# acg-team/ProGraphMSA

Hardware: AMD Instinct MI355X
Metric: DP cell-updates/sec (GCUPS) + wall-clock on 256 seqs × 1000 aa, WAG (higher is better)
Workload: dtype f32

## Files before the change

prographmsa_amd/csrc/pgm_align_kernels.h:

```cpp
#ifndef PGM_ALIGN_KERNELS_H_
#define PGM_ALIGN_KERNELS_H_

#include <hip/hip_runtime.h>
#include <math.h>
#include <type_traits>
#include "pgm_device.h"

#define PGM_NEG_INF (-INFINITY)

__device__ __forceinline__ float pgm_ls_log_add(float x, float add) {
    const float a = 2.44247459618085927548717403238913328776812604856113966238617812902399112761292613763080658235564f;
    const float b = -4.2040783745848554315883301529007786406310628696382695994938550046831869207082846248658671f;
    const float c = -0.72123729809042963774358701619456664388406302428056983119308906451199556380646306f;
    const uint32_t bits = __float_as_uint(x);
    const float e = (float)((int32_t)(bits >> 23) - 126);
    const float d = __uint_as_float(((bits << 9) >> 9) ^ 0x3f000000u);
    float t = __fdiv_rn(b, __fsub_rn(d, c));
    const float u = __fadd_rn(e, a);
    t = __fadd_rn(t, add);
    t = __fadd_rn(t, u);
    return t;
}

__device__ __forceinline__ float pgm_emission_finish(float num, float ay, float bx, float match_init) {
    float q = __fdiv_rn(num, __fmul_rn(ay, bx));
    if (q != q) q = __uint_as_float(0xFFC00000u);
    return pgm_ls_log_add(q, match_init);
}

template <int DMAX, int NODES>
__global__ void __launch_bounds__(NODES) pgm_prep_kernel(const PgmJob *__restrict__ jobs, int *__restrict__ sync, uint32_t sync_ints) {
    extern __shared__ float prep_lds[];
    {
        const uint32_t nthreads = gridDim.x * gridDim.y * gridDim.z * NODES;
        const uint32_t gid = ((blockIdx.z * gridDim.y + blockIdx.y) * gridDim.x + blockIdx.x) * NODES + threadIdx.x;
        for (uint32_t i = gid; i < sync_ints; i += nthreads) sync[i] = 0;
    }
    const PgmJob &J = jobs[blockIdx.x];
    const bool first = blockIdx.y == 0;
    const uint32_t n = first ? J.n1 : J.n2;
    const uint32_t v0 = blockIdx.z * NODES;
    if (v0 >= n) return;
    if (J.tabhdr && J.tabhdr[0] == 0) {
        const uint32_t nc = J.dim + 2u;
        bool any = n - 1u >= v0 && n - 1u < v0 + (uint32_t)NODES;
        for (uint32_t c = 0; c < nc; ++c) {
            const uint32_t r = (uint32_t)J.tabhdr[1u + (first ? 0u : nc) + c];
            any = any || (r != 0u && r - 1u >= v0 && r - 1u < v0 + (uint32_t)NODES);
        }
        if (!any) return;
    }
    const uint32_t D = J.dim, DP = J.dp, ST = D + 1;
    float *Mf = prep_lds;
    float *pif = prep_lds + D * D;
    float *nl = pif + D;
    const uint32_t nn = min((uint32_t)NODES, n - v0);
    {
        const int32_t *pp = first ? J.pp1 : J.pp2;
        const uint32_t *pc = first ? J.pc1 : J.pc2, *pu = first ? J.pu1 : J.pu2;
        const float *pv = first ? J.pv1 : J.pv2;
        PgmTbNode *rec = (first ? J.tb1 : J.tb2) + v0;
        for (uint32_t i = threadIdx.x; i < nn * PGM_TB_PK; i += NODES) {
            const uint32_t node = i / PGM_TB_PK, k = i % PGM_TB_PK;
            const int32_t eb = pp[v0 + node];
            const uint32_t cnt = (uint32_t)(pp[v0 + node + 1] - eb);
            const int32_t e = cnt == 0u ? 0 : eb + (int32_t)min(k, cnt - 1u);
            if (k == 0) rec[node].cnt = cnt;
            rec[node].c[k] = pc[e]; rec[node].v[k] = pv[e]; rec[node].u[k] = pu[e];
        }
    }
    if (!first) for (uint32_t i = threadIdx.x; i < D * D; i += NODES) Mf[i] = (float)J.M[i];
    for (uint32_t i = threadIdx.x; i < D; i += NODES) pif[i] = (float)J.pi[i];
    const double *sites = first ? J.sites1 : J.sites2;
    const uint32_t *smap = first ? J.smap1 : J.smap2;
// ... 68 lines not shown
        bool same = true;
        float vs = 0.f;
        const float g0 = (float)col[0];
        for (uint32_t k = 0; k < D; ++k) {
            const float g = (float)col[k];
            if (g != 0.0f) { ++nz; sym = k; vs = g; }
            same = same && g == g0;
        }
        uint32_t c = 255u;
        if (nz == 0u) c = D + 1u;
        else if (nz == 1u && vs == 1.0f) c = sym;
        else if (same && g0 == uni) c = D;
        cls[v] = (uint8_t)c;
        if (c == 255u) atomicOr(J.tabhdr, 1);
        else atomicCAS(J.tabhdr + 1 + (first ? 0u : D + 2u) + c, 0, (int)v + 1);
    }
}

__device__ __forceinline__ size_t pgm_cell_index(const PgmJob &J, uint32_t y, uint32_t x) {
    const uint32_t b = y / PGM_ROWS, l = PGM_HALO + (y - b * PGM_ROWS);
    return ((size_t)b * J.tsteps + (x + l)) * 64u + l;
}
__device__ __forceinline__ float4 pgm_load_cell(const PgmJob &J, uint32_t y, uint32_t x) {
    return J.cells[pgm_cell_index(J, y, x)];
}

__device__ __forceinline__ float pgm_dpp_wave_shr1(float src, float lane0_value) {
    return __int_as_float(__builtin_amdgcn_update_dpp(__float_as_int(lane0_value), __float_as_int(src), 0x138, 0xf, 0xf, false));
}

#define PGM_GLOBAL __attribute__((address_space(1)))
typedef float pgm_v4f __attribute__((ext_vector_type(4)));
template <class T> __device__ __forceinline__ T pgm_gld(const T *p) { return *(const PGM_GLOBAL T *)(uintptr_t)p; }
#define PGM_EM_TB 4
template <int DP, int RB>
__global__ void __launch_bounds__(4 * PGM_ROWS) pgm_emission_skew_kernel(const PgmJob *__restrict__ jobs) {
    typedef float pgm_v2f __attribute__((ext_vector_type(2)));
    constexpr int NT = DP / 4;
    constexpr int COLS = 64 + PGM_EM_TB * PGM_BLOCK - PGM_HALO - 1;
    constexpr int STR = DP + 1;
    __shared__ pgm_v2f tp[(COLS + 1) * STR];
    __shared__ float bq[COLS];
    const PgmJob &J = jobs[blockIdx.z];
    const uint32_t tb0 = blockIdx.x * PGM_EM_TB;
    const uint32_t rsh = J.rshift, nvb = J.nb << rsh;
    if (tb0 >= J.nblk || 4u * RB * blockIdx.y >= nvb) return;
    if (J.tabhdr && pgm_gld(J.tabhdr) == 0) return;
    auto row_of = [&](uint32_t v, uint32_t lane_) { return ((((v >> rsh) << 6) + lane_) << rsh) | (v & ((1u << rsh) - 1u)); };
    auto sblock_of = [&](uint32_t v, uint32_t tb_) { return ((((size_t)(v >> rsh) * J.nblk + tb_) << rsh) | (v & ((1u << rsh) - 1u))); };
    const uint32_t t0 = tb0 * PGM_BLOCK;
    const int cbase = (int)t0 - 63;
    if (DP == 20 && RB == 1) {
        float *const tab = (float *)tp;
        static_assert(COLS * 21 <= (COLS + 1) * STR * 2, "score table must fit the column staging area");
        __shared__ float As[32];
        const uint32_t fb0 = 4u * blockIdx.y + threadIdx.x / PGM_ROWS;
        const uint32_t fl = threadIdx.x % PGM_ROWS;
        const bool active = fb0 < nvb;
        int sym = 20;
        bool plain = true;
        float a_row = 0.f;
        if (active) {
            const uint32_t y = row_of(fb0, fl);
            const uint32_t yc = (y + 1 < J.n1) ? y : 0u;
            const float4 *src = (const float4 *)(J.g1f + (size_t)DP * yc);
            int nz = 0;
#pragma unroll
            for (int q = 0; q < NT; ++q) {
                const float4 v = src[q];
                const float vv[4] = {v.x, v.y, v.z, v.w};
#pragma unroll
                for (int u = 0; u < 4; ++u)
                    if (vv[u] != 0.0f) { ++nz; sym = 4 * q + u; plain = plain && vv[u] == 1.0f; }
            }
            plain = plain && nz <= 1;
            a_row = J.a1[yc];
        }
        if (threadIdx.x < 32) As[threadIdx.x] = 0.f;
        if (__syncthreads_and(plain ? 1 : 0)) {
            if (active) As[sym] = a_row;
            __syncthreads();
            const float mi = J.sc.match_init;
            constexpr int NE = (COLS * 21 + 4 * PGM_ROWS - 1) / (4 * PGM_ROWS);
            float tt[NE], tb2[NE];
#pragma unroll
            for (int e = 0; e < NE; ++e) {
                const int i = (int)threadIdx.x + e * 4 * PGM_ROWS;
                const int ci = i / 21, k = i % 21, c = cbase + ci;
                const bool in = i < COLS * 21 && c >= 0 && c <= (int)J.ncol;
                tb2[e] = in ? J.b2[c] : 0.f;
                tt[e] = (in && k < 20) ? J.t2[(size_t)DP * c + k] : 0.f;
            }
#pragma unroll
            for (int e = 0; e < NE; ++e) {
                const int i = (int)threadIdx.x + e * 4 * PGM_ROWS;
                if (i < COLS * 21) tab[i] = pgm_emission_finish(0.0f + tt[e], As[i % 21], tb2[e], mi);
            }
            __syncthreads();
            if (!active) return;
            PGM_GLOBAL pgm_v4f *const Sq = (PGM_GLOBAL pgm_v4f *)(uintptr_t)J.S;
            const int l = PGM_HALO + (int)fl;
#pragma unroll 1
            for (int w = 0; w < PGM_EM_TB; ++w) {
                const uint32_t tb = tb0 + w;
                if (tb >= J.nblk) break;
                float out[PGM_BLOCK];
#pragma unroll
                for (int i = 0; i < PGM_BLOCK; ++i) out[i] = tab[((int)(tb * PGM_BLOCK) + i - l - cbase) * 21 + sym];
                PGM_GLOBAL pgm_v4f *dst = Sq + (sblock_of(fb0, tb) * 64u + (uint32_t)l) * (PGM_BLOCK / 4);
#pragma unroll
                for (int q = 0; q < PGM_BLOCK / 4; ++q) dst[q] = pgm_v4f{out[4 * q], out[4 * q + 1], out[4 * q + 2], out[4 * q + 3]};
            }
            return;
        }
    }
    const float4 *t2q = (const float4 *)J.t2;
    float *tpf = (float *)tp;
    for (int i = threadIdx.x; i < (COLS + 1) * NT; i += 4 * PGM_ROWS) {
        const int ci = i / NT, q = i % NT, c = cbase + ci;
        float4 v = make_float4(0.f, 0.f, 0.f, 0.f);
        if (c >= 0 && c <= (int)J.ncol) v = t2q[(size_t)NT * c + q];
        const float vv[4] = {v.x, v.y, v.z, v.w};
#pragma unroll
        for (int u = 0; u < 4; ++u) {
            const int k = 4 * q + u;
            if (ci < COLS) tpf[2 * (ci * STR + k)] = vv[u];
            if (ci > 0) tpf[2 * ((ci - 1) * STR + k) + 1] = vv[u];
        }
    }
    for (int i = threadIdx.x; i < COLS; i += 4 * PGM_ROWS) {
        const int col = cbase + i;
        bq[i] = (col >= 0 && col <= (int)J.ncol) ? J.b2[col] : 0.f;
    }
    __syncthreads();
    const uint32_t b0 = (4u * blockIdx.y + threadIdx.x / PGM_ROWS) * RB;
    const int l = PGM_HALO + (int)(threadIdx.x % PGM_ROWS);
    if (b0 >= nvb) return;
    float gy[RB][DP], ay[RB];
#pragma unroll
    for (int r = 0; r < RB; ++r) {
        const uint32_t y = row_of(b0 + (uint32_t)r, (uint32_t)(l - PGM_HALO));
        const uint32_t yc = (y + 1 < J.n1) ? y : 0u;
        const float4 *src = (const float4 *)(J.g1f + (size_t)DP * yc);
#pragma unroll
        for (int q = 0; q < NT; ++q) {
            const float4 v = src[q];
            gy[r][4 * q] = v.x; gy[r][4 * q + 1] = v.y; gy[r][4 * q + 2] = v.z; gy[r][4 * q + 3] = v.w;
        }
        ay[r] = J.a1[yc];
    }
    const float mi = J.sc.match_init;
    const uint32_t nblk = J.nblk;
    PGM_GLOBAL pgm_v4f *const Sq = (PGM_GLOBAL pgm_v4f *)(uintptr_t)J.S;
#pragma unroll 1
    for (int w = 0; w < PGM_EM_TB; ++w) {
        const uint32_t tb = tb0 + w;
        if (tb >= nblk) break;
        float out[RB][PGM_BLOCK];
#pragma unroll
        for (int i = 0; i < PGM_BLOCK; i += 2) {
            const int ci = (int)(tb * PGM_BLOCK) + i - l - cbase;
            const pgm_v2f *tc = tp + ci * STR;
            pgm_v2f acc[RB];
#pragma unroll
            for (int r = 0; r < RB; ++r) acc[r] = pgm_v2f{0.0f, 0.0f};
#pragma unroll
            for (int k = 0; k < DP; ++k) {
                const pgm_v2f tk = tc[k];
#pragma unroll
                for (int r = 0; r < RB; ++r) {
                    const pgm_v2f g = {gy[r][k], gy[r][k]};
                    acc[r] = acc[r] + g * tk;
                }
            }
#pragma unroll
            for (int r = 0; r < RB; ++r) {
                out[r][i] = pgm_emission_finish(acc[r].x, ay[r], bq[ci], mi);
                out[r][i + 1] = pgm_emission_finish(acc[r].y, ay[r], bq[ci + 1], mi);
            }
        }
#pragma unroll
        for (int r = 0; r < RB; ++r) {
            if (b0 + (uint32_t)r < nvb) {
                PGM_GLOBAL pgm_v4f *dst = Sq + (sblock_of(b0 + (uint32_t)r, tb) * 64u + (uint32_t)l) * (PGM_BLOCK / 4);
#pragma unroll
                for (int q = 0; q < PGM_BLOCK / 4; ++q) dst[q] = pgm_v4f{out[r][4 * q], out[r][4 * q + 1], out[r][4 * q + 2], out[r][4 * q + 3]};
            }
        }
// ... 2263 lines not shown
```

prographmsa_amd/csrc/pgm_capi.hip:

```cpp
#include <hip/hip_runtime.h>

#include <algorithm>
#include <cmath>
#include <cstdio>
#include <thread>
#include <atomic>
#include <chrono>
#include <queue>
#include <cstdlib>
#include <cstring>
#include <numeric>
#include <mutex>
#include <string>
#include <unordered_set>
#include <vector>
#include <sys/mman.h>

#include "pgm_align_kernels.h"
#include "pgm_crit_kernels.h"
#include "pgm_nw_kernels.h"
#include "pgm_csprofile_kernels.h"
#include "pgm_dist_kernels.h"
#include "pgm_merge_kernels.h"
#include "pgm_pool.h"
// ... 65 lines not shown
    if (reg) { (void)hipHostUnregister(p); free(p); }
    else (void)hipHostFree(p);
}
static void slot_free(int slot, void *p) {
    if (slot == pgm_ctx::C_HIN) pinned_free(p);
    else if (slot == pgm_ctx::C_HOST) (void)hipHostFree(p);
    else (void)hipFree(p);
}

struct Arena {
    uint8_t *base = nullptr;
    size_t off = 0, end = 0;
    bool overflow = false;
    size_t put(const void *src, size_t bytes, size_t align = 16) {
        const size_t o = (off + align - 1) / align * align;
        if (o + bytes > end) { overflow = true; return 0; }
        off = o + bytes;
        if (src && bytes) memcpy(base + o, src, bytes);
        return o;
    }
};
struct DevLayout {
    size_t bytes = 0;
    size_t take(size_t b, size_t align = 256) {
        size_t off = (bytes + align - 1) / align * align;
        bytes = off + b;
        return off;
    }
};

struct pgm_align_batch {
    uint32_t njobs = 0;
    uint64_t cells = 0;
    uint32_t maxdim = 0, maxnb = 0, maxn = 0;
    std::vector<PgmJob> jobs;
    std::vector<uint32_t> order;
    uint8_t *d_in = nullptr;
    uint8_t *d_work = nullptr;
    uint8_t *d_cells = nullptr;
    uint8_t *d_out = nullptr;
    size_t cap[8] = {0, 0, 0, 0, 0, 0, 0, 0};
    uint8_t *h_out = nullptr;
    uint8_t *h_in = nullptr;
    int *h_flag = nullptr;
    uint8_t *d_small = nullptr;
    uint8_t *d_S = nullptr;
    int *d_sync = nullptr;
    size_t sync_ints = 0, s_bytes = 0;
    PgmItem *d_items = nullptr;
    uint32_t *d_lean = nullptr;
    uint32_t nlean = 0, nlean_workers = 0;
    uint32_t nbands = 0, nband_workers = 0;
    uint32_t nbands_narrow = 0, nwide_workers = 0;
    PgmItem *d_bands = nullptr;
    unsigned long long *d_times = nullptr;
    hipEvent_t ev_join_b = nullptr;
    bool crit_c3 = false, rest_c3 = false;
    uint32_t ncrit = 0, ncrit_workers = 0, ntb_c = 0;
    hipEvent_t ev_join_c = nullptr;
    uint32_t ntb_b = 0, ntb_b_workers = 0;
    uint32_t lq_off = 0, ntb = 0, ntb_workers = 0;
    int2 *d_tblist = nullptr;
    hipEvent_t ev_fork = nullptr, ev_join = nullptr;
    uint32_t test_spin_limit = 0, test_stall_job = 0xFFFFFFFFu, test_stall_band = 0;
    double acc_ms[3] = {0, 0, 0};
    uint32_t acc_n = 0;
    bool ev_pending = false;
    uint32_t nitems = 0;
    uint32_t nworkers = 0, maxnblk = 0;
    PgmJob *d_jobs = nullptr;
    uint32_t *d_order = nullptr;
    int *d_tabhdr = nullptr;
    size_t in_bytes = 0, work_bytes = 0, cell_bytes = 0, out_bytes = 0;
    std::vector<size_t> res_off, map1_off, map2_off;
    hipEvent_t ev[5] = {nullptr, nullptr, nullptr, nullptr, nullptr};
};

extern "C" {

const char *pgm_last_error(void) { return g_err.c_str(); }

int pgm_device_count(void) {
    int n = 0;
    if (hipGetDeviceCount(&n) != hipSuccess) return 0;
    return n;
}

__global__ void pgm_warm_kernel() {}

int pgm_ctx_create(int device, pgm_ctx **out) {
    if (!out) return fail(PGM_ERR_INVALID, "null out");
    *out = nullptr;
    int n = 0;
    HIPCHK(hipGetDeviceCount(&n));
    if (device < 0 || device >= n) return fail(PGM_ERR_DEVICE, "no such HIP device");
    HIPCHK(hipSetDevice(device));
    pgm_ctx *c = new pgm_ctx;
    c->device = device;
    HIPCHK(hipGetDeviceProperties(&c->prop, device));
    HIPCHK(hipStreamCreateWithFlags(&c->stream, hipStreamNonBlocking));
    HIPCHK(hipStreamCreateWithFlags(&c->stream2, hipStreamNonBlocking));
    HIPCHK(hipStreamCreateWithFlags(&c->stream3, hipStreamNonBlocking));
    {
        int lo = 0, hi = 0;
// ... 361 lines not shown
    const double w = std::min(1.0, std::max(0.0, (rsweep / t_par - 1.0) / 0.5));
    r.fl = 1.0 - 0.4 * w; r.fb = 1.0 - 0.25 * w;
    auto need = [](double cost, double t, uint32_t most) { return (uint32_t)std::min<double>(most, std::max(1.0, std::ceil(cost / t))); };
    const uint32_t band_most = (nbands + PGM_WAVES - 1) / PGM_WAVES;
    uint32_t lean = nlean ? need(lean_cost, r.fl * r.t_goal, nlean) : 0u, band = nbands ? need(band_cost, r.fb * r.t_goal, band_most) : 0u;
    uint32_t rest = nrest ? need(rest_cost, r.t_goal, nrest) : 0u;
    if (lean + band + rest > cap) {
        const double scale = (double)cap / (double)(lean + band + rest);
        auto cut = [&](uint32_t v) { return v ? std::max(1u, (uint32_t)std::floor(v * scale)) : 0u; };
        lean = cut(lean); band = cut(band); rest = cut(rest);
        while (lean + band + rest > cap) {
            uint32_t *big = &rest; if (band > *big) big = &band; if (lean > *big) big = &lean;
            if (*big <= 1u) break;
            --*big;
        }
    }
    r.rest_need = rest;
    const uint32_t left = cap > lean + band + rest ? cap - lean - band - rest : 0u;
    if (nrest) rest = std::min(nrest, rest + left);
    else if (nbands) band = std::min(band_most, band + left);
    else if (nlean) lean = std::min(nlean, lean + left);
    r.lean = lean; r.band = band; r.rest = rest;
    return r;
}

static hipError_t classify_lean_jobs(pgm_ctx *ctx, pgm_align_batch *b) {
    if (!b->d_tabhdr || b->njobs == 0) return hipSuccess;
    hipError_t e = hipMemsetAsync(b->d_tabhdr, 0, 4 * (size_t)PGM_TAB_HDR * b->njobs, ctx->stream);
    if (e != hipSuccess) return e;
    hipLaunchKernelGGL(pgm_classify_kernel, dim3(b->njobs, 2, (b->maxn + 1023) / 1024), dim3(256), 0, ctx->stream, b->d_jobs);
    return hipGetLastError();
}

#define PGM_STATUS_PENDING 0x7ffffff0
static hipError_t launch_all(pgm_ctx *ctx, pgm_align_batch *b, bool timed) {
    hipStream_t s = ctx->stream;
    hipError_t e;
    for (uint32_t i = 0; i < b->njobs; ++i) ((PgmJob::Result *)(b->h_out + b->res_off[i]))->status = PGM_STATUS_PENDING;
    if (timed && (e = hipEventRecord(b->ev[0], s)) != hipSuccess) return e;
    if (b->maxdim <= 20) {
        const size_t prep_lds = ((size_t)b->maxdim * b->maxdim + b->maxdim + 256 * ((size_t)b->maxdim + 1)) * sizeof(float);
        hipLaunchKernelGGL((pgm_prep_kernel<20, 256>), dim3(b->njobs, 2, (b->maxn + 255) / 256), dim3(256), prep_lds, s, b->d_jobs, b->d_sync, (uint32_t)b->sync_ints);
    } else {
        const size_t prep_lds = ((size_t)b->maxdim * b->maxdim + b->maxdim + 64 * ((size_t)b->maxdim + 1)) * sizeof(float);
        hipLaunchKernelGGL((pgm_prep_kernel<64, 64>), dim3(b->njobs, 2, (b->maxn + 63) / 64), dim3(64), prep_lds, s, b->d_jobs, b->d_sync, (uint32_t)b->sync_ints);
    }
    if ((e = hipGetLastError()) != hipSuccess) return e;
    if (timed && (e = hipEventRecord(b->ev[1], s)) != hipSuccess) return e;
    const dim3 eg((b->maxnblk + PGM_EM_TB - 1) / PGM_EM_TB, (b->maxnb + 3) / 4, b->njobs);
    if (b->maxdim <= 20) hipLaunchKernelGGL((pgm_emission_skew_kernel<20, 1>), eg, dim3(4 * PGM_ROWS), 0, s, b->d_jobs);
    else hipLaunchKernelGGL((pgm_emission_skew_kernel<64, 1>), eg, dim3(4 * PGM_ROWS), 0, s, b->d_jobs);
    if ((e = hipGetLastError()) != hipSuccess) return e;
    if (timed && (e = hipEventRecord(b->ev[2], s)) != hipSuccess) return e;
    const uint32_t spin_limit = b->test_spin_limit ? b->test_spin_limit : PGM_SPIN_LIMIT, stall_job = b->test_stall_job, stall_band = b->test_stall_band;
    const bool fork = b->nlean != 0;
    const bool bandk = b->nbands != 0;
    const bool tbk = (b->nitems != 0 || bandk) && (b->ntb + b->ntb_c + b->ntb_b) != 0;
    const bool critk = b->ncrit != 0;
    if ((fork || bandk || critk) && (e = hipEventRecord(b->ev_fork, s)) != hipSuccess) return e;
    if (critk && (e = hipStreamWaitEvent(ctx->stream4, b->ev_fork, 0)) != hipSuccess) return e;
    if (fork && (e = hipStreamWaitEvent(ctx->stream2, b->ev_fork, 0)) != hipSuccess) return e;
    if (bandk && (e = hipStreamWaitEvent(ctx->stream3, b->ev_fork, 0)) != hipSuccess) return e;
    const uint32_t nrest = b->nitems - b->ncrit;
    hipStream_t sc = critk ? s : ctx->stream4, sr = critk ? ctx->stream4 : s;
    auto sweep = [&](hipStream_t st, uint32_t workers, const PgmItem *list, uint32_t n, bool c3, uint32_t ticket_off) {
        if (c3) hipLaunchKernelGGL(pgm_crit_kernel, dim3(workers), dim3(64 * PGM_C3_WAVES), 0, st, b->d_jobs, list, n, b->d_sync, spin_limit, stall_job, stall_band, ticket_off);
        else hipLaunchKernelGGL(pgm_fill_kernel, dim3(workers), dim3(64 * PGM_WAVES), 0, st, b->d_jobs, list, n, b->d_sync, spin_limit, stall_job, stall_band, ticket_off);
    };
    auto tracebacks = [&](hipStream_t st, uint32_t workers, uint32_t first, uint32_t n, uint32_t lq_off, uint32_t sybase) {
        hipLaunchKernelGGL(pgm_tb_kernel, dim3(workers), dim3(64 * PGM_WAVES), 0, st, b->d_jobs, b->d_tblist + first, n, b->d_sync, b->test_spin_limit, lq_off, sybase, 1u);
    };
    if (critk) sweep(sc, b->ncrit_workers, b->d_items, b->ncrit, b->crit_c3, (uint32_t)PGM_SY_CRIT_TICKET);
    if (nrest != 0) sweep(sr, b->nworkers, b->d_items + b->ncrit, nrest, b->rest_c3, 1u);
    if ((e = hipGetLastError()) != hipSuccess) return e;
    if (fork) {
        hipLaunchKernelGGL((pgm_lean_kernel<2>), dim3(b->nlean_workers), dim3(64 * PGM_WAVES), 0, ctx->stream2, b->d_jobs, b->d_lean, b->nlean, b->d_sync, spin_limit);
        if ((e = hipGetLastError()) != hipSuccess) return e;
    }
    const uint32_t njp = (b->njobs + 3u) / 4u * 4u;
    if (bandk) {
        hipLaunchKernelGGL(pgm_band_kernel, dim3(b->nband_workers), dim3(64 * PGM_WAVES), 0, ctx->stream3, b->d_jobs, b->d_bands, b->nbands_narrow, b->nbands, b->nband_workers - b->nwide_workers, b->d_sync, spin_limit, stall_job, stall_band);
        if ((e = hipGetLastError()) != hipSuccess) return e;
        if (tbk && b->ntb_b) tracebacks(ctx->stream3, b->ntb_b_workers, b->ntb + b->ntb_c, b->ntb_b, b->lq_off + njp, 8u);
        if ((e = hipGetLastError()) != hipSuccess) return e;
// ... 56 lines not shown
        size_t E = (size_t)std::max(0, g->e_rowptr ? g->e_rowptr[n] : 0);
        if (g->r_rowptr) E += (size_t)std::max(0, g->r_rowptr[n]);
        const size_t full = side_bound_bytes(n, g->dim, E);
        return (res && res->dev_sites) ? full - n * g->dim * 8 + n * 4 + 16 : full;
    };
    auto ref_of = [&](const pgm_site_ref *r, uint32_t i) -> const pgm_site_ref * { return (r && r[i].dev_sites) ? &r[i] : nullptr; };
    std::vector<size_t> in_base(njobs + 1, 0);
    std::vector<char> two_chains(njobs, 0);
    (void)lib_pool().run(njobs, njobs >= 16 ? 16u : 1u, [&](size_t i) {
        const pgm_graph *a = g1[i], *c = g2[i];
        two_chains[i] = (a && c && a->n >= 2 && c->n >= 2 && a->e_rowptr && c->e_rowptr && a->e_col && c->e_col && a->e_val && c->e_val && graph_is_chain(a) && graph_is_chain(c)) ? 1 : 0;
    });
    uint32_t batch_dim = 0;
    for (uint32_t i = 0; i < njobs; ++i) if (g1[i]) batch_dim = std::max(batch_dim, g1[i]->dim);
    const uint32_t batch_dp = batch_dim <= 20 ? 20u : 64u;
    for (uint32_t i = 0; i < njobs; ++i) {
        const pgm_graph *a = g1[i], *c = g2[i];
        if (!a || !c || !model[i] || a->dim != c->dim || a->dim == 0 || a->dim > PGM_MAX_DIM || a->n < 2 || c->n < 2 || !model[i]->M || !model[i]->pi ||
            (!a->sites && !ref_of(res1, i)) || !a->e_rowptr || (!c->sites && !ref_of(res2, i)) || !c->e_rowptr) {
            delete b;
            return fail(PGM_ERR_INVALID, "invalid job " + std::to_string(i));
        }
        PgmJob &J = b->jobs[i];
        memset(&J, 0, sizeof J);
        J.n1 = a->n; J.n2 = c->n; J.dim = a->dim;
        J.dp = batch_dp;
        J.ncol = c->n - 1;
        J.tsteps = J.ncol + 63;
        constexpr uint32_t lean_rshift = 1u;
        J.lean = (two_chains[i] && ((uint64_t)J.tsteps * 1024u << lean_rshift) < (1ull << 30)) ? 1u : 0u;
        J.rshift = J.lean ? lean_rshift : 0u;
        J.nb = (a->n - 1 + (PGM_ROWS << J.rshift) - 1) / (PGM_ROWS << J.rshift);
        J.nblk = (J.tsteps + PGM_BLOCK - 1) / PGM_BLOCK;
        b->maxnblk = std::max(b->maxnblk, J.nblk);
        J.maxn = std::max(a->n, c->n);
        b->maxn = std::max(b->maxn, J.maxn);
        J.sc = scores[i];
        b->maxdim = std::max(b->maxdim, a->dim);
        b->maxnb = std::max(b->maxnb, J.nb << J.rshift);
        b->cells += (uint64_t)(a->n - 2) * (c->n - 2);
        Off &o = off[i];
        in_base[i + 1] = in_base[i] + side_bound(a, ref_of(res1, i)) + side_bound(c, ref_of(res2, i)) + model_bound_bytes(a->dim);
        J.keep_cells = (!J.lean || (flags & PGM_BATCH_KEEP_MATRICES)) ? 1u : 0u;
        layout_job(L, J.n1, J.n2, J.dp, J.rshift, J.lean != 0, J.keep_cells != 0, o);
        b->res_off[i] = o.res; b->map1_off[i] = o.map1; b->map2_off[i] = o.map2;
    }
    b->in_bytes = std::max<size_t>(in_base[njobs], 16);
    b->work_bytes = std::max<size_t>(L.W.bytes, 16);
    b->cell_bytes = std::max<size_t>(L.C.bytes, 16);
    b->out_bytes = std::max<size_t>(L.O.bytes, 16);
    b->s_bytes = std::max<size_t>(L.SL.bytes, 16);
    b->lq_off = (uint32_t)L.sync_ints;
    L.sync_ints += 3 * (((size_t)njobs + 3) / 4 * 4);
    const size_t sync_ints = L.sync_ints;
    b->sync_ints = sync_ints;
    hipError_t alloc_err = hipSuccess, alloc_host_err = hipSuccess;
    uint8_t *h_out_dev = nullptr;
    const bool cprof = getenv("PGM_HOST_PROFILE") != nullptr;
    auto now_ms = []() { return std::chrono::duration<double, std::milli>(std::chrono::steady_clock::now().time_since_epoch()).count(); };
    const double tc0 = now_ms();
    double tc_alloc = 0, tc_hostalloc = 0, tc_slot[6] = {0, 0, 0, 0, 0, 0};
    size_t total_bands = 0;
    for (uint32_t i = 0; i < njobs; ++i) total_bands += b->jobs[i].nb;
    DevLayout SM;
    const size_t small_sync = SM.take(sync_ints * sizeof(int)), small_jobs = SM.take(sizeof(PgmJob) * std::max(1u, njobs)),
                 small_order = SM.take(4 * (size_t)std::max(1u, njobs)), small_items = SM.take(sizeof(PgmItem) * std::max<size_t>(1, total_bands)),
                 small_lean = SM.take(4 * (size_t)std::max(1u, njobs)), small_tblist = SM.take(8 * (size_t)std::max(1u, njobs)),
                 small_bands = SM.take(sizeof(PgmItem) * std::max<size_t>(1, total_bands)), small_times = SM.take(16 * (size_t)std::max(1u, njobs) + 16);
    bool any_lean = false;
    for (uint32_t i = 0; i < njobs; ++i) any_lean = any_lean || (b->jobs[i].lean && !b->jobs[i].keep_cells);
    const size_t small_tabhdr = SM.take(any_lean ? 4 * (size_t)PGM_TAB_HDR * njobs : 16);
    const size_t small_bytes = SM.bytes;
    std::atomic<int> alloc_state(0);
    std::atomic<int> upload_err((int)hipSuccess);
    std::thread alloc_thread([&]() {
        const double ta0 = now_ms();
        hipError_t e2 = hipSetDevice(ctx->device);
        double tprev = ta0;
        auto lap = [&](int k) { const double t = now_ms(); tc_slot[k] = t - tprev; tprev = t; };
        if (e2 == hipSuccess) { e2 = cache_take(ctx, pgm_ctx::C_IN, b->in_bytes, (void **)&b->d_in, &b->cap[pgm_ctx::C_IN]); lap(0); }
        if (e2 == hipSuccess) { e2 = cache_take(ctx, pgm_ctx::C_WORK, b->work_bytes, (void **)&b->d_work, &b->cap[pgm_ctx::C_WORK]); lap(1); }
        if (e2 == hipSuccess) { e2 = cache_take(ctx, pgm_ctx::C_CELLS, b->cell_bytes, (void **)&b->d_cells, &b->cap[pgm_ctx::C_CELLS]); lap(2); }
        if (e2 == hipSuccess) { e2 = cache_take(ctx, pgm_ctx::C_OUT, b->out_bytes, (void **)&b->d_out, &b->cap[pgm_ctx::C_OUT]); lap(3); }
        if (e2 == hipSuccess) { e2 = cache_take(ctx, pgm_ctx::C_S, b->s_bytes, (void **)&b->d_S, &b->cap[pgm_ctx::C_S]); lap(4); }
        if (e2 == hipSuccess) { e2 = cache_take(ctx, pgm_ctx::C_SMALL, small_bytes, (void **)&b->d_small, &b->cap[pgm_ctx::C_SMALL]); lap(5); }
        if (e2 == hipSuccess) {
            b->d_sync = (int *)(b->d_small + small_sync);
            b->d_jobs = (PgmJob *)(b->d_small + small_jobs);
            b->d_order = (uint32_t *)(b->d_small + small_order);
            b->d_items = (PgmItem *)(b->d_small + small_items);
            b->d_lean = (uint32_t *)(b->d_small + small_lean);
            b->d_tblist = (int2 *)(b->d_small + small_tblist);
            b->d_bands = (PgmItem *)(b->d_small + small_bands);
            b->d_times = (unsigned long long *)(b->d_small + small_times);
            b->d_tabhdr = any_lean ? (int *)(b->d_small + small_tabhdr) : nullptr;
        }
        alloc_err = e2;
        alloc_state.store(e2 == hipSuccess ? 1 : -1, std::memory_order_release);
        tc_alloc = now_ms() - ta0;
        if (e2 == hipSuccess) {
            hipError_t e3 = cache_take(ctx, pgm_ctx::C_HOST, b->out_bytes + 64, (void **)&b->h_out, &b->cap[pgm_ctx::C_HOST]);
            if (e3 == hipSuccess) b->h_flag = (int *)(b->h_out + (b->out_bytes + 15) / 16 * 16);
            if (e3 == hipSuccess) e3 = hipHostGetDevicePointer((void **)&h_out_dev, b->h_out, 0);
            alloc_host_err = e3;
        }
        tc_hostalloc = now_ms() - ta0 - tc_alloc;
    });
    hipError_t e;
    if ((e = cache_take(ctx, pgm_ctx::C_HIN, b->in_bytes, (void **)&b->h_in, &b->cap[pgm_ctx::C_HIN])) != hipSuccess) {
        alloc_thread.join();
        pgm_align_batch_destroy(ctx, b);
        return fail(PGM_ERR_DEVICE, std::string("hipHostMalloc: ") + hipGetErrorString(e));
    }
    const double tc1 = now_ms();
    {
        std::atomic<int> bad(-1);
        constexpr uint32_t mode2_min_bands = 20u, mode2_min_hd = 32u;
        double longest_crit_chain = 0.0;
        for (uint32_t i = 0; i < njobs; ++i)
            longest_crit_chain = std::max(longest_crit_chain, ((double)((g1[i]->n - 1 + PGM_ROWS - 1) / PGM_ROWS - 1) * 80.0 + (double)(g2[i]->n - 1 + 63)) * 0.42);
        uint32_t promote_bands = 0xffffffffu;
        {
            double crit_load = 0.0;
            for (uint32_t i = 0; i < njobs; ++i)
                if (!b->jobs[i].lean) crit_load += (double)((g1[i]->n - 1 + PGM_ROWS - 1) / PGM_ROWS) * (double)(g2[i]->n - 1 + 63) * 0.42;
            if (crit_load <= 1.25 * (double)ctx->prop.multiProcessorCount * longest_crit_chain) promote_bands = 8u;
        }
        const uint32_t chunk_jobs = (uint32_t)std::max<size_t>(1, ((size_t)8 << 20) / std::max<size_t>(1, in_base[njobs] / std::max(1u, njobs)));
// ... 98 lines not shown
        J.ni1 = (const PgmNode2 *)(in + o.s1.ni); J.ni2 = (const PgmNode2 *)(in + o.s2.ni);
        J.xp1 = (const int32_t *)(in + o.s1.xp); J.xp2 = (const int32_t *)(in + o.s2.xp);
        J.xc1 = (const uint32_t *)(in + o.s1.xc); J.xc2 = (const uint32_t *)(in + o.s2.xc);
        J.xv1 = (const float *)(in + o.s1.xv); J.xv2 = (const float *)(in + o.s2.xv);
        J.fp1 = (const int32_t *)(in + o.s1.fp); J.fe1 = (const uint2 *)(in + o.s1.fe);
        J.ov2 = (const uint2 *)(in + o.s2.ov);
        J.pp1 = (const int32_t *)(in + o.s1.pp); J.pp2 = (const int32_t *)(in + o.s2.pp);
        J.pc1 = (const uint32_t *)(in + o.s1.pc); J.pc2 = (const uint32_t *)(in + o.s2.pc);
        J.pv1 = (const float *)(in + o.s1.pv); J.pv2 = (const float *)(in + o.s2.pv);
        J.pu1 = (const uint32_t *)(in + o.s1.pu); J.pu2 = (const uint32_t *)(in + o.s2.pu);
        J.g1f = (float *)(w + o.g1f); J.a1 = (float *)(w + o.a1);
        J.t2 = (float *)(w + o.t2); J.b2 = (float *)(w + o.aux2);
        J.map1 = (uint32_t *)(ob + o.map1); J.map2 = (uint32_t *)(ob + o.map2);
        J.mark_score = (float *)(w + o.ms); J.mark_prev = (uint32_t *)(w + o.mp);
        J.tb1 = (PgmTbNode *)(w + o.tb1); J.tb2 = (PgmTbNode *)(w + o.tb2);
        J.result = (PgmJob::Result *)(ob + o.res);
        J.hmap1 = (uint32_t *)(h_out_dev + o.map1); J.hmap2 = (uint32_t *)(h_out_dev + o.map2);
        J.hresult = (PgmJob::Result *)(h_out_dev + o.res);
        J.cells = (float4 *)(b->d_cells + o.cells);
        J.codes = (uint32_t *)(w + o.codes);
        J.endcell = (float4 *)(w + o.endcell);
        if (J.lean && !J.keep_cells && b->d_tabhdr) { J.cls1 = w + o.cls; J.cls2 = w + o.cls + J.n1; J.tabhdr = b->d_tabhdr + (size_t)PGM_TAB_HDR * i; }
        else { J.cls1 = nullptr; J.cls2 = nullptr; J.tabhdr = nullptr; }
        J.S = (float *)(b->d_S + o.S);
        J.prog = b->d_sync + o.prog;
        J.ltab = (uint16_t *)(w + o.ltab); J.lready = b->d_sync + o.lready; J.lrows = o.lrows; J.lcols = o.lcols;
        J.times = b->d_times + 2 * (size_t)i;
    }
    b->order.resize(njobs);
    std::iota(b->order.begin(), b->order.end(), 0u);
    std::stable_sort(b->order.begin(), b->order.end(), [&](uint32_t x, uint32_t y) {
        return (uint64_t)b->jobs[x].n1 * b->jobs[x].n2 > (uint64_t)b->jobs[y].n1 * b->jobs[y].n2;
    });
    std::vector<PgmItem> items;
    std::vector<uint32_t> lean_list;
    double lean_cost = 0.0, other_cost = 0.0;
    uint32_t capacity = (uint32_t)ctx->prop.multiProcessorCount;
    std::vector<PgmItem> bands;
    if (njobs) {
        struct Item { double rem, dur, gap; uint32_t job, band, count; };
        std::vector<std::vector<Item>> per_job(njobs), per_job_b(njobs), per_job_c(njobs), per_job_w(njobs);
        std::vector<double> chain_of(njobs, 0.0);
        const double lag = PGM_ROWS + 3.0 * PGM_BLOCK;
        constexpr double tau_x = 0.65, tau_c = 0.45, tau_2 = 0.6, eager = 0.7;
        constexpr double tau_3 = 0.42;
        constexpr double tau_l = 0.34;
        size_t total = 0, total_b = 0, total_w = 0;
        double rmax = 1.0, rsweep = 1.0;
        for (uint32_t q = 0; q < njobs; ++q) {
            const uint32_t i = b->order[q];
            const PgmJob &J = b->jobs[i];
            const double tau = J.crit3 ? tau_3 : (J.mode2 ? tau_2 : (J.has_extras ? tau_x : tau_c));
            const double tb = (J.has_extras ? 0.3 : 0.2) * (double)(J.n1 + J.n2);
            if (J.lean) {
                const double rounds = std::ceil((double)J.nb / PGM_WAVES), first = std::min<double>(J.nb, PGM_WAVES);
                lean_cost += tau_l * (rounds * J.tsteps + (first - 1.0) * 72.0) + 0.04 * (double)(J.n1 + J.n2);
                lean_list.push_back(i);
                continue;
            }
            const bool narrow = !J.mode2 && J.slot_bytes <= (uint32_t)(PGM_POOL / PGM_WAVES / 16 * 16);
            const bool wide = !J.mode2 && !narrow && J.slot_bytes <= (uint32_t)(PGM_POOL / PGM_WIDE_WAVES / 16 * 16);
            const bool per_band = narrow || wide;
            if (!per_band) chain_of[i] = tau * ((double)(J.nb - 1) * lag + J.tsteps);
            const uint32_t group = per_band ? 1u : J.nslots;
            for (uint32_t band = 0; band < J.nb; band += group) {
                const uint32_t cnt = std::min(group, J.nb - band);
// ... 141 lines not shown
    b->nworkers = std::max(1u, std::min(capacity, b->nitems - b->ncrit));
    b->crit_c3 = b->ncrit != 0; b->rest_c3 = b->nitems > b->ncrit;
    for (size_t k = 0; k < items.size(); ++k)
        if (!b->jobs[items[k].job].crit3) { if (k < b->ncrit) b->crit_c3 = false; else b->rest_c3 = false; }
    if (lean_list.empty()) lean_list.push_back(0u);
    if (items.size() > std::max<size_t>(1, total_bands)) {
        pgm_align_batch_destroy(ctx, b);
        return fail(PGM_ERR_DEVICE, "work list longer than the number of bands");
    }
    std::vector<int2> tblist;
    {
        std::vector<int> last_item(njobs, 0), group(njobs, 0);
        for (size_t k = 0; k < items.size(); ++k) {
            if (items[k].band + items[k].count == b->jobs[items[k].job].nb) last_item[items[k].job] = (int)k;
            if (k < b->ncrit) group[items[k].job] = 1;
        }
        if (b->nbands) for (const PgmItem &it : bands) group[it.job] = 2;
        uint32_t cnt[3] = {0, 0, 0};
        for (int pass = 0; pass < 3; ++pass)
            for (uint32_t q = 0; q < njobs; ++q) { const uint32_t i = b->order[q]; if (!b->jobs[i].lean && group[i] == pass) { tblist.push_back(make_int2((int)i, last_item[i])); ++cnt[pass]; } }
        b->ntb = cnt[0]; b->ntb_c = cnt[1]; b->ntb_b = cnt[2];
        const uint32_t all_cus = (uint32_t)std::max(1, ctx->prop.multiProcessorCount) - b->nlean_workers;
        b->ntb_workers = std::max(1u, (b->ntb_b || b->ntb_c) ? b->nworkers : all_cus);
        b->ntb_b_workers = std::max(1u, (b->ntb || b->ntb_c) ? b->nband_workers : all_cus);
        if (tblist.empty()) tblist.push_back(make_int2(0, 0));
    }
    if ((e = (hipError_t)upload_err.load()) != hipSuccess ||
        (e = hipMemcpyAsync(b->d_tblist, tblist.data(), 8 * tblist.size(), hipMemcpyHostToDevice, ctx->stream)) != hipSuccess ||
        (e = hipMemcpyAsync(b->d_jobs, b->jobs.data(), sizeof(PgmJob) * njobs, hipMemcpyHostToDevice, ctx->stream)) != hipSuccess ||
        (e = hipMemcpyAsync(b->d_order, b->order.data(), 4 * (size_t)njobs, hipMemcpyHostToDevice, ctx->stream)) != hipSuccess ||
        (e = hipMemcpyAsync(b->d_items, items.data(), sizeof(PgmItem) * items.size(), hipMemcpyHostToDevice, ctx->stream)) != hipSuccess ||
        (e = hipMemcpyAsync(b->d_lean, lean_list.data(), 4 * lean_list.size(), hipMemcpyHostToDevice, ctx->stream)) != hipSuccess ||
        (e = hipMemcpyAsync(b->d_bands, bands.data(), sizeof(PgmItem) * bands.size(), hipMemcpyHostToDevice, ctx->stream)) != hipSuccess ||
        (e = classify_lean_jobs(ctx, b)) != hipSuccess ||
        (e = hipStreamSynchronize(ctx->stream)) != hipSuccess) {
        pgm_align_batch_destroy(ctx, b);
        return fail(PGM_ERR_DEVICE, std::string("upload: ") + hipGetErrorString(e));
    }
    for (int k = 0; k < 5; ++k) (void)hipEventCreate(&b->ev[k]);
    (void)hipEventCreateWithFlags(&b->ev_fork, hipEventDisableTiming);
    (void)hipEventCreateWithFlags(&b->ev_join, hipEventDisableTiming);
    (void)hipEventCreateWithFlags(&b->ev_join_b, hipEventDisableTiming);
    (void)hipEventCreateWithFlags(&b->ev_join_c, hipEventDisableTiming);
    if (cprof)
        fprintf(stderr, "    create: sizes %.2f ms, pinned input block %.2f, flatten %.2f, wait for the allocations %.2f (device %.2f, pinned results %.2f), work list %.2f, upload of %.1f MB %.2f\n",
                tc0 - tcs, tc1 - tc0, tc2 - tc1, tc3 - tc2, tc_alloc, tc_hostalloc, tc4 - tc3, b->in_bytes / 1e6, now_ms() - tc4);
    if (cprof)
        fprintf(stderr, "    device buffers: inputs %.1f MB %.2f ms, work %.1f MB %.2f, cells %.1f MB %.2f, results %.1f MB %.2f, S %.1f MB %.2f, small %.2f\n",
                b->in_bytes / 1e6, tc_slot[0], b->work_bytes / 1e6, tc_slot[1], b->cell_bytes / 1e6, tc_slot[2], b->out_bytes / 1e6, tc_slot[3], b->s_bytes / 1e6, tc_slot[4], tc_slot[5]);
    *out = b;
    return PGM_OK;
}

int pgm_align_batch_run(pgm_ctx *ctx, pgm_align_batch *b) {
    if (!ctx || !b) return fail(PGM_ERR_INVALID, "null argument");
    if (b->njobs == 0) return PGM_OK;
    HIPCHK(hipSetDevice(ctx->device));
    HIPCHK(launch_all(ctx, b, true));
    b->ev_pending = true;
    return PGM_OK;
}

int pgm_align_batch_time(pgm_ctx *ctx, pgm_align_batch *b, int reps, float *ms_prep, float *ms_emission, float *ms_fill,
                         float *ms_traceback) {
    if (!ctx || !b || reps <= 0) return fail(PGM_ERR_INVALID, "bad argument");
    HIPCHK(hipSetDevice(ctx->device));
// ... 214 lines not shown
```

Before: 81.09.

## Launch prep and emission kernels over compacted per-job tile lists

Replaces the dense 3D grids for the prep and emission kernels, which were sized to the largest job and so launched many empty blocks for smaller jobs, with flat grids indexed by host-built tile lists. The lists cover only real tiles and are ordered by job size, with lean/tabhdr jobs placed last for emission. The emission column-block count per tile is also raised to 8 for the DP=20 path. This cuts wasted block launches and early-exit overhead. In exchange it adds host-side list construction and two small uploads, and fewer emission blocks per job could reduce parallelism.

```diff
diff --git a/prographmsa_amd/csrc/pgm_align_kernels.h b/prographmsa_amd/csrc/pgm_align_kernels.h
--- a/prographmsa_amd/csrc/pgm_align_kernels.h
+++ b/prographmsa_amd/csrc/pgm_align_kernels.h
@@ -28,18 +28,21 @@
     return pgm_ls_log_add(q, match_init);
 }
 
+struct PgmTile { uint32_t job, y, x, pad; };
+
 template <int DMAX, int NODES>
-__global__ void __launch_bounds__(NODES) pgm_prep_kernel(const PgmJob *__restrict__ jobs, int *__restrict__ sync, uint32_t sync_ints) {
+__global__ void __launch_bounds__(NODES) pgm_prep_kernel(const PgmJob *__restrict__ jobs, const PgmTile *__restrict__ tiles, int *__restrict__ sync, uint32_t sync_ints) {
     extern __shared__ float prep_lds[];
     {
-        const uint32_t nthreads = gridDim.x * gridDim.y * gridDim.z * NODES;
-        const uint32_t gid = ((blockIdx.z * gridDim.y + blockIdx.y) * gridDim.x + blockIdx.x) * NODES + threadIdx.x;
+        const uint32_t nthreads = gridDim.x * NODES;
+        const uint32_t gid = blockIdx.x * NODES + threadIdx.x;
         for (uint32_t i = gid; i < sync_ints; i += nthreads) sync[i] = 0;
     }
-    const PgmJob &J = jobs[blockIdx.x];
-    const bool first = blockIdx.y == 0;
+    const PgmTile tl = tiles[blockIdx.x];
+    const PgmJob &J = jobs[tl.job];
+    const bool first = tl.y == 0;
     const uint32_t n = first ? J.n1 : J.n2;
-    const uint32_t v0 = blockIdx.z * NODES;
+    const uint32_t v0 = tl.x * NODES;
     if (v0 >= n) return;
     if (J.tabhdr && J.tabhdr[0] == 0) {
         const uint32_t nc = J.dim + 2u;
@@ -174,19 +177,21 @@
 #define PGM_GLOBAL __attribute__((address_space(1)))
 typedef float pgm_v4f __attribute__((ext_vector_type(4)));
 template <class T> __device__ __forceinline__ T pgm_gld(const T *p) { return *(const PGM_GLOBAL T *)(uintptr_t)p; }
-#define PGM_EM_TB 4
-template <int DP, int RB>
-__global__ void __launch_bounds__(4 * PGM_ROWS) pgm_emission_skew_kernel(const PgmJob *__restrict__ jobs) {
+#define PGM_EM_TB_20 8
+#define PGM_EM_TB_64 4
+template <int DP, int RB, int TB>
+__global__ void __launch_bounds__(4 * PGM_ROWS) pgm_emission_skew_kernel(const PgmJob *__restrict__ jobs, const PgmTile *__restrict__ tiles) {
     typedef float pgm_v2f __attribute__((ext_vector_type(2)));
     constexpr int NT = DP / 4;
-    constexpr int COLS = 64 + PGM_EM_TB * PGM_BLOCK - PGM_HALO - 1;
+    constexpr int COLS = 64 + TB * PGM_BLOCK - PGM_HALO - 1;
     constexpr int STR = DP + 1;
     __shared__ pgm_v2f tp[(COLS + 1) * STR];
     __shared__ float bq[COLS];
-    const PgmJob &J = jobs[blockIdx.z];
-    const uint32_t tb0 = blockIdx.x * PGM_EM_TB;
+    const PgmTile tl = tiles[blockIdx.x];
+    const PgmJob &J = jobs[tl.job];
+    const uint32_t tb0 = tl.x, bg = tl.y;
     const uint32_t rsh = J.rshift, nvb = J.nb << rsh;
-    if (tb0 >= J.nblk || 4u * RB * blockIdx.y >= nvb) return;
+    if (tb0 >= J.nblk || 4u * RB * bg >= nvb) return;
     if (J.tabhdr && pgm_gld(J.tabhdr) == 0) return;
     auto row_of = [&](uint32_t v, uint32_t lane_) { return ((((v >> rsh) << 6) + lane_) << rsh) | (v & ((1u << rsh) - 1u)); };
     auto sblock_of = [&](uint32_t v, uint32_t tb_) { return ((((size_t)(v >> rsh) * J.nblk + tb_) << rsh) | (v & ((1u << rsh) - 1u))); };
@@ -196,7 +201,7 @@
         float *const tab = (float *)tp;
         static_assert(COLS * 21 <= (COLS + 1) * STR * 2, "score table must fit the column staging area");
         __shared__ float As[32];
-        const uint32_t fb0 = 4u * blockIdx.y + threadIdx.x / PGM_ROWS;
+        const uint32_t fb0 = 4u * bg + threadIdx.x / PGM_ROWS;
         const uint32_t fl = threadIdx.x % PGM_ROWS;
         const bool active = fb0 < nvb;
         int sym = 20;
@@ -243,7 +248,7 @@
             PGM_GLOBAL pgm_v4f *const Sq = (PGM_GLOBAL pgm_v4f *)(uintptr_t)J.S;
             const int l = PGM_HALO + (int)fl;
 #pragma unroll 1
-            for (int w = 0; w < PGM_EM_TB; ++w) {
+            for (int w = 0; w < TB; ++w) {
                 const uint32_t tb = tb0 + w;
                 if (tb >= J.nblk) break;
                 float out[PGM_BLOCK];
@@ -275,7 +280,7 @@
         bq[i] = (col >= 0 && col <= (int)J.ncol) ? J.b2[col] : 0.f;
     }
     __syncthreads();
-    const uint32_t b0 = (4u * blockIdx.y + threadIdx.x / PGM_ROWS) * RB;
+    const uint32_t b0 = (4u * bg + threadIdx.x / PGM_ROWS) * RB;
     const int l = PGM_HALO + (int)(threadIdx.x % PGM_ROWS);
     if (b0 >= nvb) return;
     float gy[RB][DP], ay[RB];
@@ -295,7 +300,7 @@
     const uint32_t nblk = J.nblk;
     PGM_GLOBAL pgm_v4f *const Sq = (PGM_GLOBAL pgm_v4f *)(uintptr_t)J.S;
 #pragma unroll 1
-    for (int w = 0; w < PGM_EM_TB; ++w) {
+    for (int w = 0; w < TB; ++w) {
         const uint32_t tb = tb0 + w;
         if (tb >= nblk) break;
         float out[RB][PGM_BLOCK];
diff --git a/prographmsa_amd/csrc/pgm_capi.hip b/prographmsa_amd/csrc/pgm_capi.hip
--- a/prographmsa_amd/csrc/pgm_capi.hip
+++ b/prographmsa_amd/csrc/pgm_capi.hip
@@ -121,7 +121,7 @@
 struct pgm_align_batch {
     uint32_t njobs = 0;
     uint64_t cells = 0;
-    uint32_t maxdim = 0, maxnb = 0, maxn = 0;
+    uint32_t maxdim = 0, maxn = 0;
     std::vector<PgmJob> jobs;
     std::vector<uint32_t> order;
     uint8_t *d_in = nullptr;
@@ -156,9 +156,11 @@
     uint32_t acc_n = 0;
     bool ev_pending = false;
     uint32_t nitems = 0;
-    uint32_t nworkers = 0, maxnblk = 0;
+    uint32_t nworkers = 0;
     PgmJob *d_jobs = nullptr;
     uint32_t *d_order = nullptr;
+    PgmTile *d_prep_tiles = nullptr, *d_em_tiles = nullptr;
+    uint32_t nprep_tiles = 0, nem_tiles = 0;
     int *d_tabhdr = nullptr;
     size_t in_bytes = 0, work_bytes = 0, cell_bytes = 0, out_bytes = 0;
     std::vector<size_t> res_off, map1_off, map2_off;
@@ -586,6 +588,17 @@
     return hipGetLastError();
 }
 
+static uint32_t prep_nodes(uint32_t dp) { return dp <= 20 ? 256u : 64u; }
+static uint32_t em_blocks(uint32_t dp) { return dp <= 20 ? (uint32_t)PGM_EM_TB_20 : (uint32_t)PGM_EM_TB_64; }
+static size_t prep_tiles_of(const PgmJob &J) {
+    const uint32_t pn = prep_nodes(J.dp);
+    return (J.n1 + pn - 1) / pn + (J.n2 + pn - 1) / pn;
+}
+static size_t em_tiles_of(const PgmJob &J) {
+    const uint32_t tb = em_blocks(J.dp);
+    return (size_t)(((J.nb << J.rshift) + 3u) / 4u) * ((J.nblk + tb - 1) / tb);
+}
+
 #define PGM_STATUS_PENDING 0x7ffffff0
 static hipError_t launch_all(pgm_ctx *ctx, pgm_align_batch *b, bool timed) {
     hipStream_t s = ctx->stream;
@@ -594,16 +607,15 @@
     if (timed && (e = hipEventRecord(b->ev[0], s)) != hipSuccess) return e;
     if (b->maxdim <= 20) {
         const size_t prep_lds = ((size_t)b->maxdim * b->maxdim + b->maxdim + 256 * ((size_t)b->maxdim + 1)) * sizeof(float);
-        hipLaunchKernelGGL((pgm_prep_kernel<20, 256>), dim3(b->njobs, 2, (b->maxn + 255) / 256), dim3(256), prep_lds, s, b->d_jobs, b->d_sync, (uint32_t)b->sync_ints);
+        hipLaunchKernelGGL((pgm_prep_kernel<20, 256>), dim3(b->nprep_tiles), dim3(256), prep_lds, s, b->d_jobs, b->d_prep_tiles, b->d_sync, (uint32_t)b->sync_ints);
     } else {
         const size_t prep_lds = ((size_t)b->maxdim * b->maxdim + b->maxdim + 64 * ((size_t)b->maxdim + 1)) * sizeof(float);
-        hipLaunchKernelGGL((pgm_prep_kernel<64, 64>), dim3(b->njobs, 2, (b->maxn + 63) / 64), dim3(64), prep_lds, s, b->d_jobs, b->d_sync, (uint32_t)b->sync_ints);
+        hipLaunchKernelGGL((pgm_prep_kernel<64, 64>), dim3(b->nprep_tiles), dim3(64), prep_lds, s, b->d_jobs, b->d_prep_tiles, b->d_sync, (uint32_t)b->sync_ints);
     }
     if ((e = hipGetLastError()) != hipSuccess) return e;
     if (timed && (e = hipEventRecord(b->ev[1], s)) != hipSuccess) return e;
-    const dim3 eg((b->maxnblk + PGM_EM_TB - 1) / PGM_EM_TB, (b->maxnb + 3) / 4, b->njobs);
-    if (b->maxdim <= 20) hipLaunchKernelGGL((pgm_emission_skew_kernel<20, 1>), eg, dim3(4 * PGM_ROWS), 0, s, b->d_jobs);
-    else hipLaunchKernelGGL((pgm_emission_skew_kernel<64, 1>), eg, dim3(4 * PGM_ROWS), 0, s, b->d_jobs);
+    if (b->maxdim <= 20) hipLaunchKernelGGL((pgm_emission_skew_kernel<20, 1, PGM_EM_TB_20>), dim3(b->nem_tiles), dim3(4 * PGM_ROWS), 0, s, b->d_jobs, b->d_em_tiles);
+    else hipLaunchKernelGGL((pgm_emission_skew_kernel<64, 1, PGM_EM_TB_64>), dim3(b->nem_tiles), dim3(4 * PGM_ROWS), 0, s, b->d_jobs, b->d_em_tiles);
     if ((e = hipGetLastError()) != hipSuccess) return e;
     if (timed && (e = hipEventRecord(b->ev[2], s)) != hipSuccess) return e;
     const uint32_t spin_limit = b->test_spin_limit ? b->test_spin_limit : PGM_SPIN_LIMIT, stall_job = b->test_stall_job, stall_band = b->test_stall_band;
@@ -726,12 +738,10 @@
         J.rshift = J.lean ? lean_rshift : 0u;
         J.nb = (a->n - 1 + (PGM_ROWS << J.rshift) - 1) / (PGM_ROWS << J.rshift);
         J.nblk = (J.tsteps + PGM_BLOCK - 1) / PGM_BLOCK;
-        b->maxnblk = std::max(b->maxnblk, J.nblk);
         J.maxn = std::max(a->n, c->n);
         b->maxn = std::max(b->maxn, J.maxn);
         J.sc = scores[i];
         b->maxdim = std::max(b->maxdim, a->dim);
-        b->maxnb = std::max(b->maxnb, J.nb << J.rshift);
         b->cells += (uint64_t)(a->n - 2) * (c->n - 2);
         Off &o = off[i];
         in_base[i + 1] = in_base[i] + side_bound(a, ref_of(res1, i)) + side_bound(c, ref_of(res2, i)) + model_bound_bytes(a->dim);
@@ -754,8 +764,12 @@
     auto now_ms = []() { return std::chrono::duration<double, std::milli>(std::chrono::steady_clock::now().time_since_epoch()).count(); };
     const double tc0 = now_ms();
     double tc_alloc = 0, tc_hostalloc = 0, tc_slot[6] = {0, 0, 0, 0, 0, 0};
-    size_t total_bands = 0;
-    for (uint32_t i = 0; i < njobs; ++i) total_bands += b->jobs[i].nb;
+    size_t total_bands = 0, nprep_tiles = 0, nem_tiles = 0;
+    for (uint32_t i = 0; i < njobs; ++i) {
+        total_bands += b->jobs[i].nb;
+        nprep_tiles += prep_tiles_of(b->jobs[i]);
+        nem_tiles += em_tiles_of(b->jobs[i]);
+    }
     DevLayout SM;
     const size_t small_sync = SM.take(sync_ints * sizeof(int)), small_jobs = SM.take(sizeof(PgmJob) * std::max(1u, njobs)),
                  small_order = SM.take(4 * (size_t)std::max(1u, njobs)), small_items = SM.take(sizeof(PgmItem) * std::max<size_t>(1, total_bands)),
@@ -764,6 +778,7 @@
     bool any_lean = false;
     for (uint32_t i = 0; i < njobs; ++i) any_lean = any_lean || (b->jobs[i].lean && !b->jobs[i].keep_cells);
     const size_t small_tabhdr = SM.take(any_lean ? 4 * (size_t)PGM_TAB_HDR * njobs : 16);
+    const size_t small_prep_tiles = SM.take(sizeof(PgmTile) * std::max<size_t>(1, nprep_tiles)), small_em_tiles = SM.take(sizeof(PgmTile) * std::max<size_t>(1, nem_tiles));
     const size_t small_bytes = SM.bytes;
     std::atomic<int> alloc_state(0);
     std::atomic<int> upload_err((int)hipSuccess);
@@ -788,6 +803,8 @@
             b->d_bands = (PgmItem *)(b->d_small + small_bands);
             b->d_times = (unsigned long long *)(b->d_small + small_times);
             b->d_tabhdr = any_lean ? (int *)(b->d_small + small_tabhdr) : nullptr;
+            b->d_prep_tiles = (PgmTile *)(b->d_small + small_prep_tiles);
+            b->d_em_tiles = (PgmTile *)(b->d_small + small_em_tiles);
         }
         alloc_err = e2;
         alloc_state.store(e2 == hipSuccess ? 1 : -1, std::memory_order_release);
@@ -952,6 +969,25 @@
     std::stable_sort(b->order.begin(), b->order.end(), [&](uint32_t x, uint32_t y) {
         return (uint64_t)b->jobs[x].n1 * b->jobs[x].n2 > (uint64_t)b->jobs[y].n1 * b->jobs[y].n2;
     });
+    std::vector<PgmTile> prep_tiles, em_tiles;
+    prep_tiles.reserve(nprep_tiles); em_tiles.reserve(nem_tiles);
+    for (uint32_t side = 2; side-- > 0;)
+        for (uint32_t q = 0; q < njobs; ++q) {
+            const uint32_t i = b->order[q], pn = prep_nodes(b->jobs[i].dp);
+            for (uint32_t x = 0; x * pn < (side ? b->jobs[i].n2 : b->jobs[i].n1); ++x) prep_tiles.push_back(PgmTile{i, side, x, 0u});
+        }
+    for (int pass = 0; pass < 2; ++pass)
+        for (uint32_t q = 0; q < njobs; ++q) {
+            const uint32_t i = b->order[q];
+            const PgmJob &J = b->jobs[i];
+            if ((J.tabhdr != nullptr) != (pass == 1)) continue;
+            const uint32_t etb = em_blocks(J.dp);
+            for (uint32_t g = 0; 4u * g < (J.nb << J.rshift); ++g)
+                for (uint32_t tb = 0; tb < J.nblk; tb += etb) em_tiles.push_back(PgmTile{i, g, tb, 0u});
+        }
+    b->nprep_tiles = (uint32_t)prep_tiles.size(); b->nem_tiles = (uint32_t)em_tiles.size();
+    if (prep_tiles.empty()) prep_tiles.push_back(PgmTile{0u, 0u, 0u, 0u});
+    if (em_tiles.empty()) em_tiles.push_back(PgmTile{0u, 0u, 0u, 0u});
     std::vector<PgmItem> items;
     std::vector<uint32_t> lean_list;
     double lean_cost = 0.0, other_cost = 0.0;
@@ -1159,6 +1195,8 @@
         (e = hipMemcpyAsync(b->d_items, items.data(), sizeof(PgmItem) * items.size(), hipMemcpyHostToDevice, ctx->stream)) != hipSuccess ||
         (e = hipMemcpyAsync(b->d_lean, lean_list.data(), 4 * lean_list.size(), hipMemcpyHostToDevice, ctx->stream)) != hipSuccess ||
         (e = hipMemcpyAsync(b->d_bands, bands.data(), sizeof(PgmItem) * bands.size(), hipMemcpyHostToDevice, ctx->stream)) != hipSuccess ||
+        (e = hipMemcpyAsync(b->d_prep_tiles, prep_tiles.data(), sizeof(PgmTile) * prep_tiles.size(), hipMemcpyHostToDevice, ctx->stream)) != hipSuccess ||
+        (e = hipMemcpyAsync(b->d_em_tiles, em_tiles.data(), sizeof(PgmTile) * em_tiles.size(), hipMemcpyHostToDevice, ctx->stream)) != hipSuccess ||
         (e = classify_lean_jobs(ctx, b)) != hipSuccess ||
         (e = hipStreamSynchronize(ctx->stream)) != hipSuccess) {
         pgm_align_batch_destroy(ctx, b);
```

Result: no change. 81.80 (median of 6 runs) (+0.9%).
